# Filippo-Galli/Split_and_merge_Gibbs_sampling

Measured on AMD Instinct MI355X. Metric: full Gibbs sweeps/sec (N-point reassign) at N=1M D=128; achieved HBM GB/s, higher is better.
Workload: dtype f64

## Files before the change

include/hdpm.h:

```cpp
#ifndef HDPM_H
#define HDPM_H

#include <stdint.h>

#ifdef __cplusplus
extern "C" {
#endif

#define HDPM_OK          0
#define HDPM_E_VALIDATE  1
#define HDPM_E_GSL       2
#define HDPM_E_PROB      3
#define HDPM_E_WALKER    4
#define HDPM_E_ARG       5
#define HDPM_E_DEVICE    6
#define HDPM_E_NODEVICE  7

typedef struct hdpm_ctx hdpm_ctx;

typedef struct {
    int32_t verbose, m, iterations, L, burnin, t, r;
    int32_t neal8, split_merge, n8_step_size, sam_step_size, thinning;
} hdpm_chain_params;

typedef struct {
    int64_t sweeps, rounds, restarts, exact_points, moves, checked_rounds, prepass_points;
    double  t_prepass_ms, t_resolve_ms, t_stats_ms, t_host_phi_ms, t_rng_ms, t_loglik_ms, t_exact_ms;
    int64_t pool_calls, pool_entries, pool_device_calls;
    double  t_pool_ms, t_pool_mt_ms, t_pool_accept_ms, t_pool_parse_ms, t_pool_values_ms;
    int64_t phi_spec_runs, phi_spec_clusters;
    int64_t prepass_timed, prepass_timed_points;
    int64_t rng_windows, rng_windows_fresh;
    int64_t listed_points;
    int64_t sm_moves;
    double  t_sm_ms, t_sm_scan_ms, t_sm_phi_ms, t_sm_terms_ms;
    int64_t phi_device_calls, phi_device_fallbacks, phi_device_last_status;
    int64_t phi_lookahead_hits, phi_lookahead_copies;
    int64_t pipe_enqueued, pipe_runs, pipe_refused, pipe_recovered;
    int64_t phi_tree_calls, phi_tree_retries;
    int64_t pool_walk_fallbacks;
    int64_t phi_dspec_launched, phi_dspec_used;
    int64_t fpg_launches;
    int64_t phi_sm_device_calls;
    int64_t phi_fallback_status_mask;
    int64_t phi_sm_window_retries;
    int64_t fpg_aborts;
    int64_t exact_mass_launches, exact_lanes_launches;
    int64_t dense_launches;
    int64_t sm_wide_scans, sm_wide_fallbacks;
    int64_t phi_fast_calls, phi_fast_handbacks;
    int64_t labels_mirrored, labels_downloaded;
    int64_t phi_state_direct;
    int64_t phi_chain_launched, phi_chain_used, phi_chain_dropped;
    int64_t pipe_auto, pipe_desync;
    int64_t sm_chain_runs, sm_chain_scans, sm_chain_resumes;
} hdpm_stats;

int         hdpm_device_count(void);
int         hdpm_ctx_create(int32_t device, hdpm_ctx** out);
void        hdpm_ctx_destroy(hdpm_ctx* ctx);
const char* hdpm_last_error(const hdpm_ctx* ctx);

int hdpm_set_data(hdpm_ctx* ctx, const uint8_t* codes, int32_t n, int32_t d, const int32_t* attrisize,
                  double gamma, const double* v, const double* w);

int hdpm_rng_set_seed(hdpm_ctx* ctx, uint32_t seed);
int hdpm_rng_set_state(hdpm_ctx* ctx, const int32_t* state625);
int hdpm_rng_get_state(const hdpm_ctx* ctx, int32_t* state625);

int hdpm_set_state(hdpm_ctx* ctx, const int32_t* c_i, int32_t K, const double* centers, const double* sigma);
int hdpm_get_state(hdpm_ctx* ctx, int32_t* c_i, int32_t* K, double* centers, double* sigma, int32_t cap);

int hdpm_set_pool(hdpm_ctx* ctx, const double* centers, const double* sigma, int64_t P);
int hdpm_get_pool(hdpm_ctx* ctx, double* centers, double* sigma, int64_t P);
int hdpm_generate_pool(hdpm_ctx* ctx, int64_t P);

int hdpm_neal8_sweep(hdpm_ctx* ctx, int32_t m);

int hdpm_update_phi(hdpm_ctx* ctx, const int32_t* cluster_indexes, int32_t n_idx);

int hdpm_compute_loglikelihood(hdpm_ctx* ctx, double* out);

int hdpm_loglik_matrix(hdpm_ctx* ctx, double* L, int32_t* H);

int hdpm_restricted_gibbs(hdpm_ctx* ctx, const int32_t* S, int32_t nS, int32_t i1, int32_t i2, int32_t t);

int hdpm_logprobgs_c_i(hdpm_ctx* ctx, const int32_t* g_c_i, const int32_t* S, int32_t nS, int32_t i1,
                       int32_t i2, double* out);

int hdpm_split_and_merge(hdpm_ctx* ctx, int32_t t, int32_t r, int32_t idx_1_sm, int32_t* accepted);

int hdpm_run_markov_chain(hdpm_ctx* ctx, const hdpm_chain_params* p, const int32_t* c_i_init,
                          int32_t* out_total_cls, int32_t* out_c_i, double* out_loglik,
                          int32_t* out_accepted, int32_t* final_ass, double* out_time_s);

int hdpm_init_chain(hdpm_ctx* ctx, const hdpm_chain_params* p, const int32_t* c_i_init);
int hdpm_iteration(hdpm_ctx* ctx, const hdpm_chain_params* p, int32_t iter, int32_t* idx_1_sm,
                   int32_t* accepted, double* loglik);
int hdpm_iterations(hdpm_ctx* ctx, const hdpm_chain_params* p, int32_t iter0, int32_t count, int32_t* idx_1_sm,
                    int32_t* accepted, double* loglik);

int hdpm_iterations_record(hdpm_ctx* ctx, const hdpm_chain_params* p, int32_t iter0, int32_t count, int32_t* idx_1_sm,
                           int32_t* accepted, double* loglik, int32_t* total_cls, int32_t* c_i, int32_t* nsaved);
int hdpm_record_take(hdpm_ctx* ctx, double* centers, double* sigmas, int64_t* nrows);

int hdpm_rng_fill_device(hdpm_ctx* ctx, int64_t count, uint32_t* out);
int hdpm_get_stats(const hdpm_ctx* ctx, hdpm_stats* out);
int hdpm_reset_stats(hdpm_ctx* ctx);
// ... 33 lines not shown
```

split_and_merge_gibbs_sampling_amd/_lib.py:

```python
from __future__ import annotations

import ctypes as C
import os
import subprocess

import numpy as np

PKG_DIR = os.path.dirname(os.path.abspath(__file__))
LIB_PATH = os.path.join(PKG_DIR, "libhdpm.so")
if os.environ.get("HDPM_LIB_VARIANT"):
    LIB_PATH = os.path.join(PKG_DIR, f"libhdpm_{os.environ['HDPM_LIB_VARIANT']}.so")
CSRC = os.path.join(PKG_DIR, "csrc")

EXPORTS = (
    "hdpm_device_count", "hdpm_ctx_create", "hdpm_ctx_destroy", "hdpm_last_error", "hdpm_set_data",
    "hdpm_rng_set_seed", "hdpm_rng_set_state", "hdpm_rng_get_state", "hdpm_set_state", "hdpm_get_state",
    "hdpm_set_pool", "hdpm_get_pool", "hdpm_generate_pool", "hdpm_neal8_sweep", "hdpm_update_phi",
    "hdpm_compute_loglikelihood", "hdpm_loglik_matrix", "hdpm_restricted_gibbs", "hdpm_logprobgs_c_i",
    "hdpm_split_and_merge", "hdpm_run_markov_chain", "hdpm_get_stats", "hdpm_reset_stats",
    "hdpm_set_debug", "hdpm_synchronize", "hdpm_drop_prepared", "hdpm_init_chain", "hdpm_iteration", "hdpm_iterations", "hdpm_iterations_record", "hdpm_record_take", "hdpm_rng_fill_device",
    "hdpm_get_pool_heads", "hdpm_set_option", "hdpm_get_option", "hdpm_debug_draw", "hdpm_debug_math",
    "hdpm_psm_build", "hdpm_psm_rows", "hdpm_psm_vi_lb",
    "hdpm_trace_build", "hdpm_trace_terms", "hdpm_trace_losses", "hdpm_trace_tables",
)

OPT_HIG_LOGSPACE = 1
OPT_PHI_DEVICE = 2
OPT_PIPE_WAIT_US = 3
OPT_FPG_WAIT_US = 4
OPT_FPG_FAIL_AT = 5
OPT_EXACT_KERNEL = 6
OPT_LAT_NEGLIGIBLE = 7
OPT_SM_WIDE_WAIT_US = 8
OPT_SM_CHAIN = 9
OPT_CAPTURE_DELAY_US = 10

STATUS = {0: "OK", 1: "E_VALIDATE", 2: "E_GSL", 3: "E_PROB", 4: "E_WALKER", 5: "E_ARG",
          6: "E_DEVICE", 7: "E_NODEVICE"}


class HdpmError(RuntimeError):
    def __init__(self, status: int, msg: str):
        super().__init__(f"hdpm {STATUS.get(status, status)}: {msg}")
        self.status = status


class ChainParams(C.Structure):
    _fields_ = [(n, C.c_int32) for n in (
        "verbose", "m", "iterations", "L", "burnin", "t", "r", "neal8", "split_merge",
        "n8_step_size", "sam_step_size", "thinning")]


class Stats(C.Structure):
    _fields_ = [(n, C.c_int64) for n in (
        "sweeps", "rounds", "restarts", "exact_points", "moves", "checked_rounds", "prepass_points")] + \
        [(n, C.c_double) for n in (
            "t_prepass_ms", "t_resolve_ms", "t_stats_ms", "t_host_phi_ms", "t_rng_ms", "t_loglik_ms",
            "t_exact_ms")] + \
        [(n, C.c_int64) for n in ("pool_calls", "pool_entries", "pool_device_calls")] + \
        [(n, C.c_double) for n in (
            "t_pool_ms", "t_pool_mt_ms", "t_pool_accept_ms", "t_pool_parse_ms", "t_pool_values_ms")] + \
        [(n, C.c_int64) for n in ("phi_spec_runs", "phi_spec_clusters", "prepass_timed", "prepass_timed_points",
                                  "rng_windows", "rng_windows_fresh", "listed_points", "sm_moves")] + \
        [(n, C.c_double) for n in ("t_sm_ms", "t_sm_scan_ms", "t_sm_phi_ms", "t_sm_terms_ms")] + \
        [(n, C.c_int64) for n in ("phi_device_calls", "phi_device_fallbacks", "phi_device_last_status",
                                  "phi_lookahead_hits", "phi_lookahead_copies", "pipe_enqueued", "pipe_runs",
                                  "pipe_refused", "pipe_recovered", "phi_tree_calls", "phi_tree_retries",
                                  "pool_walk_fallbacks", "phi_dspec_launched", "phi_dspec_used",
                                  "fpg_launches", "phi_sm_device_calls", "phi_fallback_status_mask",
                                  "phi_sm_window_retries", "fpg_aborts", "exact_mass_launches",
                                  "exact_lanes_launches", "dense_launches", "sm_wide_scans",
                                  "sm_wide_fallbacks", "phi_fast_calls", "phi_fast_handbacks",
                                  "labels_mirrored", "labels_downloaded", "phi_state_direct",
                                  "phi_chain_launched", "phi_chain_used", "phi_chain_dropped",
                                  "pipe_auto", "pipe_desync", "sm_chain_runs", "sm_chain_scans",
                                  "sm_chain_resumes")]

    def as_dict(self):
        return {k: getattr(self, k) for k, _ in self._fields_}


def build(force: bool = False) -> str:
    srcs = [os.path.join(CSRC, f) for f in os.listdir(CSRC)]
    stale = force or not os.path.exists(LIB_PATH) or \
        max(os.path.getmtime(s) for s in srcs) > os.path.getmtime(LIB_PATH)
    if stale:
        subprocess.run(["make", "-s", "-C", CSRC], check=True)
    return LIB_PATH


_lib = None


def lib():
    global _lib
    if _lib is not None:
        return _lib
    if not os.path.exists(LIB_PATH):
        raise ImportError(f"libhdpm.so not built ({LIB_PATH}); run __graft_entry__.build()")
    L = C.CDLL(LIB_PATH)
    vp, i32, i64, f64 = C.c_void_p, C.c_int32, C.c_int64, C.c_double
    P = C.POINTER
    sig = {
        "hdpm_device_count": ([], C.c_int),
        "hdpm_ctx_create": ([i32, P(vp)], C.c_int),
        "hdpm_ctx_destroy": ([vp], None),
        "hdpm_last_error": ([vp], C.c_char_p),
        "hdpm_set_data": ([vp, vp, i32, i32, vp, f64, vp, vp], C.c_int),
        "hdpm_rng_set_seed": ([vp, C.c_uint32], C.c_int),
        "hdpm_rng_set_state": ([vp, vp], C.c_int),
        "hdpm_rng_get_state": ([vp, vp], C.c_int),
        "hdpm_set_state": ([vp, vp, i32, vp, vp], C.c_int),
        "hdpm_get_state": ([vp, vp, P(i32), vp, vp, i32], C.c_int),
        "hdpm_set_pool": ([vp, vp, vp, i64], C.c_int),
        "hdpm_get_pool": ([vp, vp, vp, i64], C.c_int),
        "hdpm_generate_pool": ([vp, i64], C.c_int),
        "hdpm_neal8_sweep": ([vp, i32], C.c_int),
        "hdpm_update_phi": ([vp, vp, i32], C.c_int),
        "hdpm_compute_loglikelihood": ([vp, P(f64)], C.c_int),
        "hdpm_loglik_matrix": ([vp, vp, vp], C.c_int),
        "hdpm_restricted_gibbs": ([vp, vp, i32, i32, i32, i32], C.c_int),
        "hdpm_logprobgs_c_i": ([vp, vp, vp, i32, i32, i32, P(f64)], C.c_int),
        "hdpm_split_and_merge": ([vp, i32, i32, i32, P(i32)], C.c_int),
        "hdpm_run_markov_chain": ([vp, P(ChainParams), vp, vp, vp, vp, vp, vp, vp], C.c_int),
        "hdpm_get_stats": ([vp, P(Stats)], C.c_int),
        "hdpm_init_chain": ([vp, P(ChainParams), vp], C.c_int),
        "hdpm_iteration": ([vp, P(ChainParams), i32, P(i32), P(i32), P(f64)], C.c_int),
        "hdpm_iterations": ([vp, P(ChainParams), i32, i32, P(i32), vp, vp], C.c_int),
        "hdpm_iterations_record": ([vp, P(ChainParams), i32, i32, P(i32), vp, vp, vp, vp, P(i32)], C.c_int),
# ... 30 lines not shown
```

split_and_merge_gibbs_sampling_amd/csrc/engine.cpp:

```cpp
#include <hip/hip_runtime.h>

#include <algorithm>
#include <cctype>
#include <atomic>
#include <chrono>
#include <condition_variable>
#include <cstdlib>
#include <functional>
#include <mutex>
#include <pthread.h>
#include <sched.h>
#include <dirent.h>
#include <dlfcn.h>
#include <execinfo.h>
#include <csignal>
#include <unistd.h>
#include <cmath>
#include <cstdio>
#include <cstring>
#include <memory>
#include <string>
#include <thread>
#include <unordered_map>
#include <vector>
// ... 727 lines not shown
    DevBuf<int32_t> gj, gn, cidx;
    PinBuf<int64_t> h_starts;
    int64_t walk_fallbacks = 0;
    DevBuf<PoolClass> cls;
    DevBuf<int> runs;
    DevBuf<int32_t> att;
    DevBuf<uint64_t> gtab;
    DevBuf<int> err;
    PinBuf<int> h_err;
  } pg;

  PinBuf<uint32_t> h_raw;
  DevBuf<uint32_t> d_raw;
  DevBuf<double> d_L;
  int Ecap = 0;
  DevBuf<double> d_margin;
  DevBuf<int> d_rowpos;
  DevBuf<int> d_list, d_cnt, d_dense, d_dense_total, d_spec, d_boff;
  DevBuf<double> d_spec_rad;
  DevBuf<int4> d_rq;
  DevBuf<uint64_t> d_csum;
  DevBuf<unsigned> d_hist_part;
  DevBuf<long long> d_rprof;
  DevBuf<int> d_fpg;
  DevBuf<int> d_wide_ctr;
  DevBuf<int> d_warm;
  DevBuf<unsigned int> d_lmask;
  bool kernels_warm = false;
  int fpg_grid_cache[65] = {0};
  int fpg_grid_m = -1;
  int& fpg_grid(int lcap, int m) {
    if (m != fpg_grid_m) {
      std::fill(fpg_grid_cache, fpg_grid_cache + 65, 0);
      fpg_grid_m = m;
    }
    return fpg_grid_cache[lcap];
  }
  PinBuf<int> h_ctl;
  int par = 0;
  hipEvent_t ev_res[2] = {nullptr, nullptr};
  size_t ctl_stride() const { return kCtlInts + 3 * (size_t)scap; }
  ResolveCtl* ctl_at(int q) { return reinterpret_cast<ResolveCtl*>(h_ctl.p + (size_t)q * ctl_stride()); }
  PinBuf<PipeSlot> h_pipe;
  DevBuf<PipeGate> d_pipe;
  struct PreSweep {
    bool active = false;
    bool round_ok = false;
    int par = 0, buf = -1, m = 0;
    bool track = false;
    bool dev = false;
    uint64_t gen[2] = {0, 0};
    std::chrono::steady_clock::time_point t_enq;
    bool au = false;
  } pre;
  bool pipe_auto = true;
  int pre_dev_decision() {
    if (!pre.active || !pre.au) return 0;
    const int* w = &h_pipe.p[pre.par].dev;
    const auto t0 = std::chrono::steady_clock::now();
    for (int polls = 0;; ++polls) {
      const int v = __atomic_load_n(w, __ATOMIC_ACQUIRE);
      if (v != 0) return v;
      HostPool::spin_pause();
      if ((polls & 1023) == 1023 && std::chrono::steady_clock::now() - t0 > std::chrono::seconds(5)) {
        return 2;
      }
    }
  }
  long long pipe_limit_ticks = 200000000LL;
  bool pipe_host_check = true;
  long long fpg_limit_ticks = 200000000LL;
  int fpg_fail_at = 0;
  bool fpg_skip = false;
  int last_xpath = 0;
  int exact_pref = 0;
  double lat_negl = kLatNegligible;
  long long sm_wide_ticks = 5000000;
  int sm_chain_mode = [] {
    const char* e = std::getenv("HDPM_SM_CHAIN");
    return (e && e[0] == '1') ? 1 : 0;
  }();
  bool deep_ok = false;
  static constexpr size_t kCtlInts = 16;
  static_assert(sizeof(ResolveCtl) <= kCtlInts * sizeof(int), "control block");
  PinBuf<uint8_t> h_stage_buf[3];
  hipEvent_t ev_stage_buf[3] = {nullptr, nullptr, nullptr};
  int stage_fill = 0, stage_last = 1;
  int stage_hold = -1;
  struct { bool active = false, dev = false; int buf = 0, nent = 0; } commit_later;
  DevBuf<uint8_t> d_stage;

  DevBuf<unsigned> d_freq, d_freq2, d_freq_m;
  bool freq_dev_valid = false;
  bool recount_only() const { return (debug & 16) != 0; }
  uint64_t freq_d2h_version = 0;
  DevBuf<int> d_mlog, d_mcount;
  PinBuf<unsigned> h_freq;
  DevBuf<unsigned char> d_mask;
  PinBuf<unsigned char> h_mask;
  StreamAhead phi_stream;
  int64_t phi_prefetch = 4096;
  DevBuf<double> d_partial;
  PinBuf<double> h_partial;

  hdpm_stats stats{};
  int64_t launch_count = 0;
  bool round_timed = false, round_fine = false;
  int64_t round_points = 0;
  bool pre_timed[2] = {false, false};
  hipEvent_t ev_pp[2][2] = {{nullptr, nullptr}, {nullptr, nullptr}};
  int debug = 0;
  std::vector<std::pair<const char*, std::chrono::steady_clock::time_point>> trace;
  void mark(const char* what) {
    if (debug & 34) trace.emplace_back(what, std::chrono::steady_clock::now());
  }
  std::vector<std::pair<std::string, double>> trace_sum;
  std::vector<std::vector<float>> trace_smp;
  void trace_add(const std::string& name, double us) {
    size_t q = 0;
    while (q < trace_sum.size() && trace_sum[q].first != name) ++q;
    if (q == trace_sum.size()) {
      trace_sum.emplace_back(name, 0.0);
      trace_smp.emplace_back();
    }
    trace_sum[q].second += us;
    trace_smp[q].push_back((float)us);
  }
  int64_t trace_iters = 0, trace_alloc0 = -1, trace_slow = 0;
  char spec_line[192] = {0};
  std::unordered_map<uint64_t, bool> beta_cache;

  SmWork sm;
  std::vector<double> sp;
  std::vector<int> sperm;

  ~Ctx() {
    PoolScope scope(hpool);
    try {
      cancel_ahead();
    } catch (...) {
    }
// ... 419 lines not shown
      for (int b = 0; b < wb; ++b)
        if ((code >> b) & 1u) out[b * Ws + (j >> 6)] |= 1ull << (j & 63);
      A += (long double)tab[2 * j];
      sc += (long double)std::max(std::fabs(tab[2 * j]), std::fabs(tab[2 * j + 1]));
      const double dj = tab[2 * j] - tab[2 * j + 1];
      dmax = std::max(dmax, dj);
      dmin = std::min(dmin, dj);
    }
    const double delta = dmax > 0 ? dmax / ((1 << kQ) - 1) : 0.0;
    for (int j = 0; j < d; ++j) {
      const double dj = tab[2 * j] - tab[2 * j + 1];
      int q = delta > 0 ? (int)std::floor(dj / delta) : 0;
      q = std::min(std::max(q, 0), (1 << kQ) - 1);
      while (q > 0 && delta * q > dj) --q;
      while (q < (1 << kQ) - 1 && delta * (q + 1) <= dj) ++q;
      for (int b = 0; b < kQ; ++b)
        if ((q >> b) & 1) out[(wb + b) * Ws + (j >> 6)] |= 1ull << (j & 63);
    }
    double* s = reinterpret_cast<double*>(out + (wb + kQ) * Ws);
    s[0] = (double)A;
    s[1] = delta;
    s[2] = dmin > 0 ? dmin : 0.0;
    s[3] = (double)sc;
  }

  void ensure_slots(int need) {
    if (need <= scap) return;
    int nc = std::max(need, std::max(2 * scap, 64));
    d_counts.ensure(nc, true, stream);
    d_sol.ensure(nc, true, stream);
    d_los.ensure(nc, true, stream);
    d_src.ensure(nc, true, stream);
    d_slot_codes.ensure((size_t)nc * dp, true, stream);
    d_slot_tab.ensure((size_t)nc * 2 * d, true, stream);
    d_slot_bnd.ensure((size_t)nc * bw, true, stream);
    d_freq.ensure((size_t)nc * d * mmax, true, stream);
    d_freq2.ensure((size_t)nc * d * mmax);
    scap = nc;
  }

  UploadLayout stage_begin(int nent) {
    const UploadLayout L = upload_layout(nent, dp, d, bw);
    auto pick = [&] {
      int f = 0;
      while (f < 3 && (f == stage_last || f == stage_hold || (commit_later.active && f == commit_later.buf))) ++f;
      return f;
    };
    int f = pick();
    if (f >= 3) {
      flush_commit();
      f = pick();
    }
    stage_fill = f;
    hipEvent_t& ev = ev_stage_buf[stage_fill];
    if (!ev) HIPCHK(hipEventCreateWithFlags(&ev, hipEventDisableTiming));
    HIPCHK(hipEventSynchronize(ev));
    PinBuf<uint8_t>& hb = h_stage_buf[stage_fill];
    if (hb.n < L.bytes) hb.ensure(L.bytes + L.bytes / 2 + 4096, hipHostMallocCoherent);
    d_stage.ensure(L.bytes);
    return L;
  }
  uint8_t* stage_ptr() { return h_stage_buf[stage_fill].p; }
  void stage_entry(const UploadLayout& L, int r, int k) {
    uint8_t* st = stage_ptr();
    double* tt = (double*)(st + L.off_tab) + (size_t)r * 2 * d;
    tables_for(&h_center[(size_t)k * d], &h_sigma[(size_t)k * d], st + L.off_codes + (size_t)r * dp, tt);
    bounds_for(&h_center[(size_t)k * d], tt, (uint64_t*)(st + L.off_bnd) + (size_t)r * bw);
    ((int*)(st + L.off_counts))[r] = h_counts[k];
    ((int*)(st + L.off_slot))[r] = k;
  }
  void stage_commit(const UploadLayout& L, int nent, bool full) {
    if (stage_hold == stage_fill) stage_hold = -1;
    HIPCHK(hipMemcpyAsync(d_stage.p, stage_ptr(), L.bytes, hipMemcpyHostToDevice, stream));
    HIPCHK(hipEventRecord(ev_stage_buf[stage_fill], stream));
    stage_last = stage_fill;
    stage_full = full;
    HIPCHK(launch_scatter_clusters(d_stage.p, nent, dp, d, bw, full ? 1 : 0, d_slot_codes.p, d_slot_tab.p,
                                   d_slot_bnd.p, d_counts.p, d_sol.p, d_los.p, d_src.p, stream));
  }

  bool defer_commit = false;
  void flush_commit() {
    if (!commit_later.active) return;
    commit_later.active = false;
    if (commit_later.dev) {
      commit_later.dev = false;
      scatter_dev_stage(commit_later.nent);
      return;
    }
    stage_fill = commit_later.buf;
    stage_commit(upload_layout(commit_later.nent, dp, d, bw), commit_later.nent, true);
  }

  void stage_upload(const std::vector<int>* which) {
    const int nent = which ? (int)which->size() : K;
    if (nent == 0) return;
    const UploadLayout L = stage_begin(nent);
    pool_for(nent, [&](int r) { stage_entry(L, r, which ? (*which)[r] : r); });
    stage_commit(L, nent, which == nullptr);
  }

  void upload_clusters() {
    ensure_slots(K + 2);
    stage_upload(nullptr);
    tables_dirty = false;
  }
// ... 819 lines not shown
    if (!host_spec()) {
      dspec_launch();
      mark("ahead.dspec");
    }
    if (resolve_smem_bytes(std::min(scap, K + 2), m, K + m <= 64 ? 1 : 0) <= 160 * 1024) {
      par ^= 1;
      ahead.par = par;
      ahead.track = freq_dev_valid;
      sweep_buffers(ahead.track, m);
      mark("ahead.buf");
      if (launch) {
        if (launch_round(0, K, m, ahead.raw, ahead.track) == kOk) ahead.launched = true;
      } else if (!(debug & 131072)) {
        HIPCHK(hipEventRecord(ev[7], stream));
        if (launch_round(0, K, m, ahead.raw, ahead.track, kRoundPrefix) == kOk) ahead.prefix = true;
      }
    }
    if (sweep_first && host_spec()) {
      spec_launch();
      mark("ahead.spec");
    }
  }
  void cancel_ahead() {
    pre_release();
    if (!ahead.active) return;
    ahead.active = false;
    if (ahead.launched) {
      (void)hipStreamSynchronize(stream);
      have_state = false;
      err = "a prepared sweep was abandoned";
    }
    if (spec.ran) {
      if (!spec.joined && pj_open) (void)pj_finish();
      spec.ran = false;
    }
    dspec.ran = false;
    dnext.ran = false;
    phi_stream.n = 0;
    pend.active = false;
    rng = ahead.saved;
  }

  int last_sweep_rounds = 0, last_sweep_moves = -1;

  void pre_enqueue(int m, bool track) {
    const int q = 1 - par;
    if (h_pipe.n < 2) h_pipe.ensure(2, hipHostMallocCoherent);
    d_pipe.ensure(2);
    sweep_buffers(track, m);
    __atomic_store_n(&h_pipe.p[q].flag, 0, __ATOMIC_RELEASE);
    __atomic_store_n(&h_pipe.p[q].dev, 0, __ATOMIC_RELEASE);
    h_pipe.p[q].raw = nullptr;
    h_pipe.p[q].raw_dev = nullptr;
    const bool dev = !host_spec();
    const uint64_t lo = dev ? dspec.pos : spec.pos;
    const uint64_t hi = lo + (uint64_t)(dev ? dspec.pl.need : 2 * phi_prefetch) + (uint64_t)n * (m + 1);
    int whole = -1;
    for (int k = 0; k < 2; ++k) {
      const RngWindow& w = win[k];
      if (w.valid && w.epoch == rng.epoch && w.start_pos <= lo && hi <= w.start_pos + (uint64_t)w.count &&
          (whole < 0 || w.start_pos < win[whole].start_pos))
        whole = k;
    }
    for (int k = 0; k < 2; ++k) {
      pre.gen[k] = ~0ull;
      const RngWindow& w = win[k];
      if (whole >= 0 ? k == whole
                     : (w.valid && w.epoch == rng.epoch && w.start_pos < hi && lo < w.start_pos + (uint64_t)w.count)) {
        HIPCHK(hipStreamWaitEvent(stream, w.done, 0));
        pre.gen[k] = w.gen;
      }
    }
    static const bool auto_env_off = [] {
      const char* e = std::getenv("HDPM_PIPE_AUTO");
      return e && e[0] == '0';
    }();
    PipeAuto au{};
    const bool labels_from_device = record_now && !host_c_valid;
    if (dev && pipe_auto && !auto_env_off && dspec.ran && dspec.fast && dspec.chain && whole >= 0 &&
        !labels_from_device) {
      const RngWindow& w = win[whole];
      au = PipeAuto{dspec.chain, w.raw.p, (int64_t)w.start_pos, w.count, (int64_t)n * (m + 1), 1};
    }
    if (dev) HIPCHK(hipStreamWaitEvent(stream, dspec.ev, 0));
    HIPCHK(launch_pipe_wait(&h_pipe.p[q], ctl_at(par), ctl_at(q), n, &d_pipe.p[q], pipe_limit_ticks, stream, au));
    pre.au = au.on != 0;
    pre.t_enq = std::chrono::steady_clock::now();
    pre.active = true;
    pre.par = q;
    pre.dev = dev;
    pre.buf = dev ? -1 : spec.stage_buf;
    pre.m = m;
    pre.track = track;
    pre.round_ok = false;
    d_csum.ensure((size_t)K * (bw + 2));
    d_wide_ctr.ensure(4);
    int* zero = nullptr;
    if (mcount_clear && K > 0) {
      zero = d_mcount.p;
      mcount_clear = false;
    }
    if (dev) {
      HIPCHK(launch_scatter_clusters(dspec.stage, K, dp, d, bw, 1, d_slot_codes.p, d_slot_tab.p, d_slot_bnd.p,
                                     d_counts.p, d_sol.p, d_los.p, d_src.p, stream, &d_pipe.p[q].gate, d_csum.p,
                                     d_logn.p, zero, d_wide_ctr.p));
      phd_release(stream);
    } else {
      HIPCHK(launch_scatter_clusters(h_stage_buf[pre.buf].p, K, dp, d, bw, 1, d_slot_codes.p, d_slot_tab.p,
                                     d_slot_bnd.p, d_counts.p, d_sol.p, d_los.p, d_src.p, stream, &d_pipe.p[q].gate,
                                     d_csum.p, d_logn.p, zero, d_wide_ctr.p));
    }
    summary_by_scatter = true;
    pre.round_ok = launch_round(0, K, m, nullptr, track, kRoundAll, &d_pipe.p[q], q) == kOk;
    summary_by_scatter = false;
    if (!dev) HIPCHK(hipEventRecord(ev_stage_buf[pre.buf], stream));
    stats.pipe_enqueued++;
  }
  void pre_release() {
    if (!pre.active) return;
    if (pre_dev_decision() == 1) {
      (void)hipStreamSynchronize(stream);
      have_state = false;
      err = "a sweep went ahead on the device after the host released it";
      stats.pipe_desync++;
    }
    pre.active = false;
    __atomic_store_n(&h_pipe.p[pre.par].flag, 2, __ATOMIC_RELEASE);
  }
  bool pipe_go(int m) {
    const bool went = pre_dev_decision() == 1;
    const bool agree = pre.active && pre.round_ok && pre.m == m && commit_later.active && last_sweep_rounds == 1 &&
                       last_sweep_moves == 0 && !tables_dirty;
    if (went && !(agree && pre.dev && commit_later.dev && freq_dev_valid && freq_version == labels_version)) {
      (void)hipStreamSynchronize(stream);
      have_state = false;
      err = "a sweep went ahead on the device where the host would not have";
      stats.pipe_desync++;
      pre.active = false;
      return false;
    }
    if (!went) {
      if (!agree) return false;
      if (pre.dev ? (!commit_later.dev || !dspec_on()) : (commit_later.dev || commit_later.buf != pre.buf || !host_spec()))
        return false;
      if (!(freq_dev_valid && freq_version == labels_version)) return false;
      if (pipe_host_check &&
          std::chrono::duration<double, std::micro>(std::chrono::steady_clock::now() - pre.t_enq).count() >
              (double)pipe_limit_ticks * 0.01 * 0.25) {
        stats.pipe_refused++;
        return false;
      }
    }
    rng_sync();
    const Rng saved = rng;
    const uint32_t* raw = device_draws((int64_t)n * (m + 1));
    PipeSlot& sl = h_pipe.p[pre.par];
    if (went) {
      raw = __atomic_load_n(&sl.raw_dev, __ATOMIC_ACQUIRE);
      stats.pipe_auto++;
    } else {
      bool waited = false;
      for (int k = 0; k < 2; ++k)
        if (win[k].gen == pre.gen[k] && raw >= win[k].raw.p && raw < win[k].raw.p + win[k].count) waited = true;
      if (!waited) {
        pend.active = false;
        phidev.valid = false;
        rng = saved;
        return false;
      }
      __atomic_store_n(&sl.raw, raw, __ATOMIC_RELAXED);
      __atomic_store_n(&sl.flag, 1, __ATOMIC_RELEASE);
    }
    pre.active = false;
    mark("go");
    ahead.saved = saved;
    ahead.raw = raw;
    ahead.m = m;
    ahead.lv = labels_version;
    ahead.launched = true;
    ahead.prefix = false;
    ahead.track = pre.track;
    ahead.par = pre.par;
    ahead.piped = true;
    ahead.active = true;
    stats.prepass_points += n;
    stats.pipe_runs++;
    commit_later.active = false;
    if (pre.dev) {
      commit_later.dev = false;
      stage_full = false;
      if (!dspec_promote(m)) dspec_launch();
      dnext_launch(m);
    } else {
      stage_last = pre.buf;
      stage_full = true;
      if (stage_hold == pre.buf) stage_hold = -1;
      spec_launch();
    }
    mark("ahead.spec");
    return true;
  }

  int neal8_sweep(int m) {
    const bool use_ahead = ahead.active && ahead.m == m && ahead.lv == labels_version && !tables_dirty;
    if (!use_ahead) cancel_ahead();
    if (!have_state) { err = "no state"; return kArg; }
    if (P <= 0) { err = "no latent pool"; return kArg; }
    if (m <= 0) { err = "m must be positive"; return kArg; }
    {
      if (!host_c_valid || host_c_device) {  }
      else {
        std::vector<char> seen(K + 1, 0);
        int u = 0;
        for (int i = 0; i < n; ++i) {
          const int c = h_c[i];
          if (c >= K) { cancel_ahead(); err = "State validation failed: inconsistent cluster count"; return kValidate; }
          if (!seen[c]) { seen[c] = 1; u++; }
        }
        if (u != K) { cancel_ahead(); err = "State validation failed: inconsistent cluster count"; return kValidate; }
      }
    }
    if (tables_dirty) upload_clusters();
    const bool spec_go = freq_dev_valid && freq_version == labels_version && !(debug & 128) && !recount_only() &&
                         host_spec();
    const bool freq_before_ok = freq_version == labels_version && !recount_only();
    const bool dspec_go = freq_dev_valid && freq_version == labels_version && !recount_only() && dspec_on();
    if (!use_ahead) {
      spec.ran = false;
      dspec.ran = false;
    }
    spec.lv = 0;
    labels_version++;
    const int K0 = K;
    int sweep_moves = 0;
    const bool hc_before = host_c_valid;
    std::vector<uint8_t> old_center = h_center;
    std::vector<double> old_sigma = h_sigma;

    auto tr0 = std::chrono::steady_clock::now();
    const size_t nraw = (size_t)n * (m + 1);
    const uint32_t* d_sweep_raw = use_ahead ? ahead.raw : device_draws((int64_t)nraw);
    const bool ahead_launched = use_ahead && ahead.launched;
    const bool ahead_prefix = use_ahead && ahead.prefix && !ahead.launched;
    const bool ahead_piped = ahead_launched && ahead.piped;
    if (ahead_launched || ahead_prefix) par = ahead.par;
    else par ^= 1;
    ahead.active = false;
    mark("draws");
    struct SpecGuard {
      Ctx* c;
      ~SpecGuard() {
        if (c->spec.ran && !c->spec.joined && c->pj_open) {
          (void)c->pj_finish();
          c->spec.ran = false;
        }
      }
    } spec_guard{this};
    if (spec_go && !use_ahead) spec_launch();
    else if (dspec_go && !use_ahead) dspec_launch();
    stats.t_rng_ms += std::chrono::duration<double, std::milli>(std::chrono::steady_clock::now() - tr0).count();

    int nslots = K;
    int p = 0;
    bool end_queued = false;
    const int64_t rounds0 = stats.rounds;
    const bool launched_ahead = ahead_launched;
    const bool track = (launched_ahead || ahead_prefix) ? ahead.track : (freq_dev_valid && !recount_only());
    if (!launched_ahead && !ahead_prefix) sweep_buffers(track, m);
    while (p < n) {
      if (!(launched_ahead && stats.rounds == rounds0)) {
        const int part = (ahead_prefix && stats.rounds == rounds0) ? kRoundResolve : kRoundAll;
        const int lst = launch_round(p, nslots, m, d_sweep_raw, track, part);
        if (lst) return lst;
        end_queued = last_sweep_moves > 0;
        if (end_queued) launch_sweep_end(scap - 2, track);
      } else {
        end_queued = false;
      }
      mark("launched");
      if (stats.rounds == rounds0) {
        if (deep_ok && (host_spec() ? (spec.ran && spec.K == K) : (dspec.ran && dspec.K == K)) && track &&
            last_sweep_moves == 0 && !(debug & 4194304)) {
          pre_enqueue(m, track);
          mark("pre");
        }
        if (spec.ran) spec_join();
        else if (host_spec()) prefill_phi_stream();
      }
      mark("prefill");
      HIPCHK(hipEventSynchronize(ev_res[par]));
      mark("resolved");
      const bool piped_round = ahead_piped && stats.rounds == rounds0;
      if (piped_round ? pre_timed[par] : round_timed) {
        float t1 = 0;
        if (piped_round) round_points = n;
        HIPCHK(hipEventElapsedTime(&t1, piped_round ? ev_pp[par][0] : ev[0], piped_round ? ev_pp[par][1] : ev[1]));
        stats.t_prepass_ms += t1;
        stats.prepass_timed++;
        stats.prepass_timed_points += round_points;
      }
      if (round_fine && !piped_round) {
        float t2 = 0, t3 = 0;
        HIPCHK(hipEventElapsedTime(&t3, ev[1], ev[5]));
        HIPCHK(hipEventElapsedTime(&t2, ev[5], ev[2]));
        stats.t_exact_ms += t3;
        stats.t_resolve_ms += t2;
      }
      stats.rounds++;
      const ResolveCtl c = *ctl_at(par);
      if (c.status == kPipeOff && piped_round) {
        if (pre.dev || stage_last < 0 || !stage_full) {
          upload_clusters();
        } else {
          stage_fill = stage_last;
          stage_commit(upload_layout(K, dp, d, bw), K, true);
        }
        if (track) mcount_clear = true;
        stats.pipe_recovered++;
        continue;
      }
      if (pre.active && (c.status || c.next < n || c.moves)) pre_release();
      last_sweep_rounds = (int)(stats.rounds - rounds0);
      if ((debug & 2) && last_fp && last_fpg) {
        long long tp[16];
        HIPCHK(hipMemcpy(tp, d_rprof.p, sizeof(tp), hipMemcpyDeviceToHost));
        std::fprintf(stderr,
                     "[resolve_fpg] G %d: %lld listed in %lld windows, %lld rounds; init %.2f us, rounds %.2f us, drift / "
                     "re-test / commit %.2f us, in grid barriers %.2f us, total %.2f us\n",
                     last_fpg, tp[9], tp[8], tp[5], (tp[1] - tp[0]) / 100.0, tp[3] / 100.0, tp[4] / 100.0, tp[2] / 100.0,
                     (tp[7] - tp[0]) / 100.0);
      } else if ((debug & 2) && last_fp) {
        long long tp[16];
        HIPCHK(hipMemcpy(tp, d_rprof.p, sizeof(tp), hipMemcpyDeviceToHost));
        std::fprintf(stderr,
                     "[resolve_fp] init %.2f us, %lld listed in %lld chunks: rounds %lld (%.2f us), drift / re-test / "
                     "commit %.2f us, %lld stops (%.2f us), total %.2f us; in rounds: counts %.2f us, ballots %.2f us, "
                     "evaluations (slowest wave) %.2f us, %lld evaluations, %lld own draws (row loads + draws: %.2f us, summed over waves)\n",
                     (tp[1] - tp[0]) / 100.0, tp[9], tp[8], tp[5], tp[3] / 100.0, tp[4] / 100.0, tp[6], tp[2] / 100.0,
                     (tp[7] - tp[0]) / 100.0, tp[10] / 100.0, tp[11] / 100.0, tp[12] / 100.0, tp[14], tp[15], tp[13] / 100.0);
      } else if (debug & 2) {
        long long tp[16];
        HIPCHK(hipMemcpy(tp, d_rprof.p, sizeof(tp), hipMemcpyDeviceToHost));
        std::fprintf(stderr,
                     "[resolve] init %.2f us, batches %.2f us, decided points %lld in %.2f us (exact decisions "
                     "%.2f us, state updates %.2f us, re-tests %.2f us over %lld points; block mode: %lld blocks), "
                     "total %.2f us\n",
                     (tp[1] - tp[0]) / 100.0, tp[3] / 100.0, tp[6], tp[4] / 100.0, tp[12] / 100.0, tp[14] / 100.0,
                     tp[13] / 100.0, tp[15], tp[5], (tp[7] - tp[0]) / 100.0);
      }
      stats.exact_points += c.exact;
      stats.listed_points += c.listed;
      last_exact = c.exact;
      last_listed = c.listed;
      if (p == 0 || last_density < 0)
        last_density = (double)(c.uncertain >= 0 ? c.uncertain : c.listed) / (double)std::max(1, n - p);
      stats.moves += c.moves;
      sweep_moves += c.moves;
      stats.checked_rounds += c.checked;
      last_unsettled = c.checked || (c.restart && c.next < n);
      if (c.aborted && !c.status) {
        stats.fpg_aborts++;
        fpg_skip = true;
// ... 1752 lines not shown
  }
  h_center.assign((size_t)K * d, 0);
  h_sigma.assign((size_t)K * d, 0.0);
  for (int k = 0; k < K; ++k) sample_center_uniform(&h_center[(size_t)k * d]);
  for (int k = 0; k < K; ++k) {
    int st = sample_sigma(v.data(), w.data(), &h_sigma[(size_t)k * d]);
    if (st) { err = "rhig failed"; return st; }
  }
  recount();
  upload_labels();
  upload_clusters();
  have_state = true;
  int st = update_phi(nullptr, 0);
  if (st) return st;
  return generate_pool((int64_t)n * p->m * p->thinning);
}

int Ctx::iteration(const hdpm_chain_params* p, int iter, int* idx_1_sm, int* accepted, double* ll, bool launch_next,
                   int32_t* labels_out) {
  int st;
  *accepted = 0;
  trace.clear();
  mark("start");
  const bool n8 = p->neal8 && iter % p->n8_step_size == 0;
  const bool sm_now = p->split_merge && iter % p->sam_step_size == 0;
  const bool next_n8 = p->neal8 && (iter + 1) % p->n8_step_size == 0;
  const bool early = n8 && !sm_now && next_n8 && iter % 1000 != 0 && !(debug & 2097152);
  if (!n8) cancel_ahead();
  if (n8) {
    deep_ok = early && launch_next && !(debug & 4194304);
    record_now = labels_out != nullptr;
    st = neal8_sweep(p->m);
    deep_ok = false;
    record_now = false;
    if (st) {
      pre_release();
      return st;
    }
    if (labels_out) capture_labels();
    defer_commit = early;
    st = update_phi(nullptr, 0);
    defer_commit = false;
    if (st) {
      pre_release();
      flush_commit();
      return st;
    }
  }
  bool prepared = false;
  if (pre.active) {
    if (early && launch_next && pipe_go(p->m)) prepared = true;
    else pre_release();
  }
  if (!prepared && early && commit_later.active && freq_version == labels_version && !(debug & 4) && !tables_dirty) {
    prepare_next_sweep(p->m, launch_next);
    prepared = true;
  }
  flush_commit();
  if (sm_now) {
    const auto t0 = std::chrono::steady_clock::now();
    st = split_and_merge(p->t, p->r, *idx_1_sm, accepted);
    stats.t_sm_ms += std::chrono::duration<double, std::milli>(std::chrono::steady_clock::now() - t0).count();
    stats.sm_moves++;
    if (st) return st;
    *idx_1_sm = (*idx_1_sm + 1) % n;
  }
  if (iter % 1000 == 0) {
    st = generate_pool((int64_t)n * p->m * p->thinning);
    if (st) return st;
  }
  st = compute_loglikelihood(ll);
  mark("loglik");
  if (!st && labels_out) {
    if (sm_now || !n8) capture_labels();
    std::memcpy(labels_out, h_c.data(), (size_t)n * 4);
  }
  if (!st && next_n8 && !prepared) {
    prepare_next_sweep(p->m, launch_next);
    prepared = true;
  }
  if (prepared && ahead.active && host_spec()) phi_lookahead();
  mark("ahead");
  if ((debug & 32) && trace.size() > 1) {
    if (trace_alloc0 < 0) trace_alloc0 = g_dev_allocs.load();
    for (size_t k = 1; k < trace.size(); ++k) {
      const double us = std::chrono::duration<double, std::micro>(trace[k].second - trace[k - 1].second).count();
      trace_add(trace[k].first, us);
    }
    const double tot = std::chrono::duration<double, std::micro>(trace.back().second - trace.front().second).count();
    trace_add("total", tot);
    if (tot > 180.0 && trace_slow++ < 12) {
      std::string line = "[slow iteration " + std::to_string(trace_iters) + "]";
      for (size_t k = 1; k < trace.size(); ++k) {
        char buf[64];
        std::snprintf(buf, sizeof(buf), " %s %.0f", trace[k].first,
                      std::chrono::duration<double, std::micro>(trace[k].second - trace[k - 1].second).count());
        line += buf;
      }
      std::fprintf(stderr, "%s%s\n", line.c_str(), spec_line);
    }
    trace_iters++;
  }
  if ((debug & 2) && trace.size() > 1) {
    std::string line = "[iter]";
    for (size_t k = 1; k < trace.size(); ++k) {
      char buf[96];
// ... 752 lines not shown
```

split_and_merge_gibbs_sampling_amd/csrc/kernels.hip:

```cpp
#include <hip/hip_runtime.h>

#include <algorithm>
#include <cfloat>
#include <cmath>
#include <cstdlib>
#include <cstdio>

#include "glibc_math.hpp"
#include "kernels.hpp"

namespace hdpm {

int device_cus() {
  static int cache[64] = {0};
  int dev = 0;
  if (hipGetDevice(&dev) != hipSuccess || dev < 0 || dev >= 64) dev = 0;
  int c = __atomic_load_n(&cache[dev], __ATOMIC_RELAXED);
  if (c <= 0) {
    if (hipDeviceGetAttribute(&c, hipDeviceAttributeMultiprocessorCount, dev) != hipSuccess || c <= 0) c = 256;
    __atomic_store_n(&cache[dev], c, __ATOMIC_RELAXED);
  }
  return c;
}

// ... 3781 lines not shown
  } else if (a.fp) {
    const size_t lds = resolve_fp_lds_bytes(a.lcap, a.m);
    if (a.K + a.m <= 24) HDPM_LAUNCH(k_resolve_fp<24>, dim3(1), dim3(kFpThreads), lds, s, a);
    else if (a.K + a.m <= 32) HDPM_LAUNCH(k_resolve_fp<32>, dim3(1), dim3(kFpThreads), lds, s, a);
    else HDPM_LAUNCH(k_resolve_fp<64>, dim3(1), dim3(kFpThreads), lds, s, a);
  } else if (a.blocks)
    HDPM_LAUNCH(k_resolve_blk, dim3(1), dim3(kWave), resolve_lds_bytes(a.lcap, a.m, 1), s, a);
  else
    HDPM_LAUNCH(k_resolve, dim3(1), dim3(kWave), resolve_lds_bytes(a.lcap, a.m, 0, a.S + a.m), s, a);
  return hipGetLastError();
}

hipError_t launch_relabel(int* c, const int* los, int n, const ResolveCtl* ctl, hipStream_t s) {
  HDPM_LAUNCH(k_relabel, dim3((n + kBlock - 1) / kBlock), dim3(kBlock), 0, s, c, los, n, ctl);
  return hipGetLastError();
}

hipError_t launch_apply_moves(const int* mlog, const int* mcount, int grid, const uint8_t* codes_t, int d, int nq,
                              int mmax, unsigned int* freq, const ResolveCtl* ctl, int n, int nslots, hipStream_t s) {
  const int ls = std::min(nslots, (int)(64 * 1024 / ((size_t)d * mmax * 4)));
  if (ls >= 2) {
    HDPM_LAUNCH(k_apply_moves_lds, dim3(512), dim3(256), (size_t)ls * d * mmax * 4, s, mlog, mcount, codes_t, d,
                       nq, mmax, freq, ctl, n, ls);
    return hipGetLastError();
  }
  HDPM_LAUNCH(k_apply_moves, dim3(std::max(1, std::min(grid, 4096))), dim3(kWave), 0, s, mlog, mcount, codes_t,
                     d, nq, mmax, freq, ctl, n);
  return hipGetLastError();
}

hipError_t launch_freq_gather(const unsigned int* freq, const int* sol, int Kmax, int fs, unsigned int* out,
                              const ResolveCtl* ctl, int n, hipStream_t s) {
  const int64_t work = (int64_t)std::max(Kmax, 1) * fs;
  HDPM_LAUNCH(k_freq_gather, dim3((unsigned)std::min<int64_t>(1024, (work + 255) / 256)), dim3(256), 0, s, freq,
                     sol, fs, out, ctl, n);
  return hipGetLastError();
}

hipError_t launch_finish_sweep(int* counts, int* sol, int* los, int* src, int cap, const ResolveCtl* ctl, int n,
                               hipStream_t s) {
  HDPM_LAUNCH(k_finish_sweep, dim3(1), dim3(1024), (size_t)(2 * cap) * 4, s, counts, sol, los, src, ctl, n);
  return hipGetLastError();
}

__global__ void k_pipe_wait(PipeSlot* slot, const ResolveCtl* prev, ResolveCtl* own, int n, PipeGate* g,
                            long long limit, PipeAuto au) {
  if (threadIdx.x != 0) return;
  if (au.on) {
    const volatile ResolveCtl* c = prev;
    const int cok = __hip_atomic_load(&au.chain->ok, __ATOMIC_ACQUIRE, __HIP_MEMORY_SCOPE_AGENT);
    const int64_t end =
        (int64_t)__hip_atomic_load(reinterpret_cast<const uint64_t*>(&au.chain->end), __ATOMIC_RELAXED, __HIP_MEMORY_SCOPE_AGENT);
    const int64_t r = end - au.win_start;
    const bool ok = cok == 1 && c->status == 0 && c->next >= n && c->moves == 0 && r >= 0 && r + au.sweep_len <= au.win_count;
    if (ok) {
      const uint32_t* raw = au.win_raw + r;
      g->raw = raw;
      g->status = 4;
      g->gate = 1;
      __hip_atomic_store(reinterpret_cast<uint64_t*>(&slot->raw_dev), reinterpret_cast<uint64_t>(raw), __ATOMIC_RELAXED,
                         __HIP_MEMORY_SCOPE_SYSTEM);
      __hip_atomic_store(&slot->dev, 1, __ATOMIC_RELEASE, __HIP_MEMORY_SCOPE_SYSTEM);
      return;
    }
    __hip_atomic_store(&slot->dev, 2, __ATOMIC_RELEASE, __HIP_MEMORY_SCOPE_SYSTEM);
  }
  const long long t0 = wall_clock64();
  int f = 0;
  for (;;) {
    f = __hip_atomic_load(&slot->flag, __ATOMIC_RELAXED, __HIP_MEMORY_SCOPE_SYSTEM);
    if (f != 0) {
      __builtin_amdgcn_fence(__ATOMIC_ACQUIRE, "");
      break;
    }
    if (wall_clock64() - t0 > limit) {
      f = 3;
      break;
    }
    __builtin_amdgcn_s_sleep(8);
  }
  const volatile ResolveCtl* c = prev;
  const bool ok = f == 1 && c->status == 0 && c->next >= n && c->moves == 0;
  const uint64_t rw =
      __hip_atomic_load(reinterpret_cast<const uint64_t*>(&slot->raw), __ATOMIC_ACQUIRE, __HIP_MEMORY_SCOPE_SYSTEM);
  g->raw = ok ? reinterpret_cast<const uint32_t*>(rw) : nullptr;
  g->status = f;
  g->gate = ok ? 1 : 0;
  if (!ok) {
    volatile ResolveCtl* o = own;
    o->status = kPipeOff;
    o->next = 0;
    o->aborted = 0;
    o->uncertain = -1;
  }
}
hipError_t launch_pipe_wait(PipeSlot* slot, const ResolveCtl* prev, ResolveCtl* own, int n, PipeGate* g,
                            long long limit, hipStream_t s, const PipeAuto& au) {
  HDPM_LAUNCH(k_pipe_wait, dim3(1), dim3(64), 0, s, slot, prev, own, n, g, limit, au);
  return hipGetLastError();
}

hipError_t launch_scatter_clusters(const uint8_t* stage, int nent, int dp, int d, int bw, int full, uint8_t* codes,
                                   double* tab, uint64_t* bnd, int* counts, int* sol, int* los, int* src,
                                   hipStream_t s, const int* gate, uint64_t* csum, const double* logn, int* zero,
                                   int* wide_ctr) {
  if (csum && !full) return hipErrorInvalidValue;
  const int64_t work = (int64_t)nent * std::max(2 * d, std::max(dp, bw + 2));
  const int nb = (int)std::max<int64_t>(1, std::min<int64_t>(1024, (work + 255) / 256));
  const ScatterSummary sum{csum, logn, zero, wide_ctr};
  HDPM_LAUNCH(k_scatter_clusters, dim3(nb), dim3(256), 0, s, stage, nent, dp, d, bw, full, codes, tab, bnd,
                     counts, sol, los, src, gate, sum);
  return hipGetLastError();
}

size_t hist_partial_words(const HistArgs& a, int* nbx_out, int* kc_out, int* tpb_out) {
  const int64_t per_label = (int64_t)a.mmax * a.d * 4;
  const int64_t budget = 96 * 1024 - (int64_t)(kHistBlock / kWave) * a.W * 64 * 8 - per_label;
  const int kc = budget > 0 ? (int)std::min<int64_t>(a.K, budget / per_label) : 0;
  const int64_t ntiles = ((int64_t)a.n + 63) / 64;
  const int tpb = (int)std::max<int64_t>(16, (ntiles + 255) / 256);
  const int nbx = (int)((ntiles + tpb - 1) / tpb);
  *nbx_out = nbx;
  *kc_out = kc;
  *tpb_out = tpb;
  if (kc <= 0 || a.W > 8) return 0;
  const int ny = (a.K + kc - 1) / kc;
  return (size_t)ny * nbx * kc * a.mmax * a.d;
}

hipError_t launch_hist(const HistArgs& a0, hipStream_t s) {
  HistArgs a = a0;
  int nbx, kc, tpb;
  const size_t pw = hist_partial_words(a, &nbx, &kc, &tpb);
  const hipError_t e = hipMemsetAsync(a.freq, 0, (size_t)a.K * a.d * a.mmax * 4, s);
  if (e != hipSuccess) return e;
  if (pw > 0 && a.partial && a.xpk) {
    a.KC = kc;
    a.tiles_per_block = tpb;
    const int ny = (a.K + kc - 1) / kc;
    const size_t hbytes = (((size_t)(kc + 1) * a.mmax * a.d * 4 + 15) / 16) * 16;
    const size_t lds = hbytes + (size_t)(kHistBlock / kWave) * a.W * 64 * 8;
    HDPM_LAUNCH(k_hist_packed, dim3(nbx, ny), dim3(kHistBlock), lds, s, a);
    const int hsize = kc * a.mmax * a.d;
    HDPM_LAUNCH(k_hist_reduce, dim3((hsize + 255) / 256, ny, kHistReduceSplit), dim3(256), 0, s, a, nbx);
  } else {
    const int64_t nt = (int64_t)a.n * a.nq;
    HDPM_LAUNCH(k_hist_global, dim3((nt + kBlock - 1) / kBlock), dim3(kBlock), 0, s, a);
// ... 776 lines not shown
```

Measured before the change: 8060.

## Release the enqueued-ahead host-spec sweep early, before the current round resolves

Adds an early-go path for the host-speculation pipeline. When the host has already prepared the next sweep's phi stream and reserved its RNG window, it sets the wait slot's flag and raw pointer right after enqueueing, so the device's pipe_wait kernel can proceed without a later host round-trip. The wait kernel now reports its decision in the slot in the non-auto case as well, and staging-buffer reuse is guarded by tracking which pipe slot still reads each buffer. The added consistency checks (draw-pointer match, quiet-sweep confirmation, desync handling) cost extra host logic and risk invalidating state whenever the speculation disagrees with what the host later computes.

```diff
diff --git a/include/hdpm.h b/include/hdpm.h
--- a/include/hdpm.h
+++ b/include/hdpm.h
@@ -54,6 +54,7 @@
     int64_t phi_chain_launched, phi_chain_used, phi_chain_dropped;
     int64_t pipe_auto, pipe_desync;
     int64_t sm_chain_runs, sm_chain_scans, sm_chain_resumes;
+    int64_t pipe_early, pipe_early_ran, pipe_early_off;
 } hdpm_stats;
 
 int         hdpm_device_count(void);
diff --git a/split_and_merge_gibbs_sampling_amd/_lib.py b/split_and_merge_gibbs_sampling_amd/_lib.py
--- a/split_and_merge_gibbs_sampling_amd/_lib.py
+++ b/split_and_merge_gibbs_sampling_amd/_lib.py
@@ -74,7 +74,7 @@
                                   "labels_mirrored", "labels_downloaded", "phi_state_direct",
                                   "phi_chain_launched", "phi_chain_used", "phi_chain_dropped",
                                   "pipe_auto", "pipe_desync", "sm_chain_runs", "sm_chain_scans",
-                                  "sm_chain_resumes")]
+                                  "sm_chain_resumes", "pipe_early", "pipe_early_ran", "pipe_early_off")]
 
     def as_dict(self):
         return {k: getattr(self, k) for k, _ in self._fields_}
diff --git a/split_and_merge_gibbs_sampling_amd/csrc/engine.cpp b/split_and_merge_gibbs_sampling_amd/csrc/engine.cpp
--- a/split_and_merge_gibbs_sampling_amd/csrc/engine.cpp
+++ b/split_and_merge_gibbs_sampling_amd/csrc/engine.cpp
@@ -803,18 +803,29 @@
     uint64_t gen[2] = {0, 0};
     std::chrono::steady_clock::time_point t_enq;
     bool au = false;
+    bool early = false;
+    const uint32_t* early_raw = nullptr;
+    bool early_went = false;
   } pre;
   bool pipe_auto = true;
   int pre_dev_decision() {
-    if (!pre.active || !pre.au) return 0;
-    const int* w = &h_pipe.p[pre.par].dev;
+    if (!pre.active || !(pre.au || pre.early)) return 0;
+    return slot_dev_decision(pre.par);
+  }
+  int slot_dev_decision(int q) {
+    const int* w = &h_pipe.p[q].dev;
     const auto t0 = std::chrono::steady_clock::now();
     for (int polls = 0;; ++polls) {
       const int v = __atomic_load_n(w, __ATOMIC_ACQUIRE);
       if (v != 0) return v;
       HostPool::spin_pause();
       if ((polls & 1023) == 1023 && std::chrono::steady_clock::now() - t0 > std::chrono::seconds(5)) {
-        return 2;
+        (void)hipStreamSynchronize(stream);
+        have_state = false;
+        err = "the wait kernel of a sweep enqueued ahead did not report its decision";
+        stats.pipe_desync++;
+        const int v2 = __atomic_load_n(w, __ATOMIC_ACQUIRE);
+        return v2 != 0 ? v2 : 2;
       }
     }
   }
@@ -838,6 +849,7 @@
   hipEvent_t ev_stage_buf[3] = {nullptr, nullptr, nullptr};
   int stage_fill = 0, stage_last = 1;
   int stage_hold = -1;
+  int stage_pipe_busy[3] = {0, 0, 0};
   struct { bool active = false, dev = false; int buf = 0, nent = 0; } commit_later;
   DevBuf<uint8_t> d_stage;
 
@@ -1363,6 +1375,12 @@
       f = pick();
     }
     stage_fill = f;
+    if (stage_pipe_busy[f]) {
+      const int q = stage_pipe_busy[f] - 1;
+      if (ev_res[q]) HIPCHK(hipEventSynchronize(ev_res[q]));
+      else HIPCHK(hipStreamSynchronize(stream));
+      stage_pipe_busy[f] = 0;
+    }
     hipEvent_t& ev = ev_stage_buf[stage_fill];
     if (!ev) HIPCHK(hipEventCreateWithFlags(&ev, hipEventDisableTiming));
     HIPCHK(hipEventSynchronize(ev));
@@ -2288,6 +2306,9 @@
     __atomic_store_n(&h_pipe.p[q].dev, 0, __ATOMIC_RELEASE);
     h_pipe.p[q].raw = nullptr;
     h_pipe.p[q].raw_dev = nullptr;
+    pre.early = false;
+    pre.early_raw = nullptr;
+    pre.early_went = false;
     const bool dev = !host_spec();
     const uint64_t lo = dev ? dspec.pos : spec.pos;
     const uint64_t hi = lo + (uint64_t)(dev ? dspec.pl.need : 2 * phi_prefetch) + (uint64_t)n * (m + 1);
@@ -2349,8 +2370,39 @@
     summary_by_scatter = true;
     pre.round_ok = launch_round(0, K, m, nullptr, track, kRoundAll, &d_pipe.p[q], q) == kOk;
     summary_by_scatter = false;
-    if (!dev) HIPCHK(hipEventRecord(ev_stage_buf[pre.buf], stream));
+    if (!dev) stage_pipe_busy[pre.buf] = q + 1;
     stats.pipe_enqueued++;
+  }
+  void pipe_early_go(int m, bool track, bool freq_before_ok) {
+    static const bool env_off = [] {
+      const char* e = std::getenv("HDPM_PIPE_EARLY");
+      return e && e[0] == '0';
+    }();
+    if (env_off || !pre.active || !pre.round_ok || pre.dev || pre.au || pre.m != m) return;
+    if (!pipe_host_check || (record_now && !host_c_valid)) return;
+    const StreamAhead& sa = phi_stream;
+    if (!(deep_ok && host_spec() && !(debug & 128))) return;
+    if (!(spec.ran && spec.joined && K > 0 && spec.K == K && spec.nvalid == K)) return;
+    if (!(spec.pos == rng.pos && spec.epoch == rng.epoch && sa.n > 0 && sa.start.pos == spec.pos)) return;
+    if (!(spec.stage_buf >= 0 && spec.stage_buf == stage_hold && spec.stage_buf == pre.buf)) return;
+    if (!(track && freq_dev_valid && freq_before_ok)) return;
+    if (std::chrono::duration<double, std::micro>(std::chrono::steady_clock::now() - pre.t_enq).count() >
+        (double)pipe_limit_ticks * 0.01 * 0.25)
+      return;
+    const uint64_t pos = spec.pos + (uint64_t)spec.off[K];
+    const int64_t len = (int64_t)n * (m + 1);
+    int wk = -1;
+    for (int k = 0; k < 2; ++k)
+      if (covers(win[k], pos, len) && (wk < 0 || win[k].start_pos < win[wk].start_pos)) wk = k;
+    if (wk < 0 || win[wk].gen != pre.gen[wk]) return;
+    const uint32_t* raw = win[wk].raw.p + (pos - win[wk].start_pos);
+    PipeSlot& sl = h_pipe.p[pre.par];
+    pre.early = true;
+    pre.early_raw = raw;
+    __atomic_store_n(&sl.raw, raw, __ATOMIC_RELAXED);
+    __atomic_store_n(&sl.flag, 1, __ATOMIC_RELEASE);
+    stats.pipe_early++;
+    mark("early_go");
   }
   void pre_release() {
     if (!pre.active) return;
@@ -2362,12 +2414,16 @@
     }
     pre.active = false;
     __atomic_store_n(&h_pipe.p[pre.par].flag, 2, __ATOMIC_RELEASE);
+    if (pre.buf >= 0) stage_pipe_busy[pre.buf] = 0;
   }
   bool pipe_go(int m) {
-    const bool went = pre_dev_decision() == 1;
+    const bool early = pre.active && pre.early;
+    const bool went = early ? pre.early_went : pre_dev_decision() == 1;
     const bool agree = pre.active && pre.round_ok && pre.m == m && commit_later.active && last_sweep_rounds == 1 &&
                        last_sweep_moves == 0 && !tables_dirty;
-    if (went && !(agree && pre.dev && commit_later.dev && freq_dev_valid && freq_version == labels_version)) {
+    const bool same_tables = pre.dev ? (pre.au && commit_later.dev)
+                                     : (pre.early && !commit_later.dev && commit_later.buf == pre.buf && host_spec());
+    if (went && !(agree && same_tables && freq_dev_valid && freq_version == labels_version)) {
       (void)hipStreamSynchronize(stream);
       have_state = false;
       err = "a sweep went ahead on the device where the host would not have";
@@ -2391,7 +2447,16 @@
     const Rng saved = rng;
     const uint32_t* raw = device_draws((int64_t)n * (m + 1));
     PipeSlot& sl = h_pipe.p[pre.par];
-    if (went) {
+    if (went && early) {
+      if (raw != pre.early_raw) {
+        (void)hipStreamSynchronize(stream);
+        have_state = false;
+        err = "a sweep went ahead on the device with other draws than the host reserved";
+        stats.pipe_desync++;
+        pre.active = false;
+        return false;
+      }
+    } else if (went) {
       raw = __atomic_load_n(&sl.raw_dev, __ATOMIC_ACQUIRE);
       stats.pipe_auto++;
     } else {
@@ -2432,9 +2497,17 @@
       stage_full = true;
       if (stage_hold == pre.buf) stage_hold = -1;
       spec_launch();
+      if (early) pipe_early_confirm(pre.par);
     }
     mark("ahead.spec");
     return true;
+  }
+  void pipe_early_confirm(int q) {
+    if (slot_dev_decision(q) == 1 && have_state) return;
+    (void)hipStreamSynchronize(stream);
+    have_state = false;
+    err = "the host followed an early go that the device did not take";
+    stats.pipe_desync++;
   }
 
   int neal8_sweep(int m) {
@@ -2504,6 +2577,7 @@
     const bool track = (launched_ahead || ahead_prefix) ? ahead.track : (freq_dev_valid && !recount_only());
     if (!launched_ahead && !ahead_prefix) sweep_buffers(track, m);
     while (p < n) {
+      bool enqueued = false;
       if (!(launched_ahead && stats.rounds == rounds0)) {
         const int part = (ahead_prefix && stats.rounds == rounds0) ? kRoundResolve : kRoundAll;
         const int lst = launch_round(p, nslots, m, d_sweep_raw, track, part);
@@ -2519,13 +2593,17 @@
             last_sweep_moves == 0 && !(debug & 4194304)) {
           pre_enqueue(m, track);
           mark("pre");
+          enqueued = true;
         }
         if (spec.ran) spec_join();
         else if (host_spec()) prefill_phi_stream();
+        if (enqueued) pipe_early_go(m, track, freq_before_ok);
       }
       mark("prefill");
       HIPCHK(hipEventSynchronize(ev_res[par]));
       mark("resolved");
+      for (int& b : stage_pipe_busy)
+        if (b == par + 1) b = 0;
       const bool piped_round = ahead_piped && stats.rounds == rounds0;
       if (piped_round ? pre_timed[par] : round_timed) {
         float t1 = 0;
@@ -2544,6 +2622,25 @@
       }
       stats.rounds++;
       const ResolveCtl c = *ctl_at(par);
+      if (pre.active && pre.early && enqueued) {
+        if (!c.status && c.next >= n && !c.moves) {
+          pre.early_went = true;
+          stats.pipe_early_ran++;
+        } else {
+          const int dv = pre_dev_decision();
+          pre.active = false;
+          if (pre.buf >= 0) stage_pipe_busy[pre.buf] = 0;
+          if (!have_state) return kArg;
+          if (dv == 1) {
+            (void)hipStreamSynchronize(stream);
+            have_state = false;
+            err = "a sweep went ahead on the device behind a sweep that was not quiet";
+            stats.pipe_desync++;
+            return kArg;
+          }
+          stats.pipe_early_off++;
+        }
+      }
       if (c.status == kPipeOff && piped_round) {
         if (pre.dev || stage_last < 0 || !stage_full) {
           upload_clusters();
@@ -4402,6 +4499,7 @@
     if (early && launch_next && pipe_go(p->m)) prepared = true;
     else pre_release();
   }
+  if (!have_state) return kArg;
   if (!prepared && early && commit_later.active && freq_version == labels_version && !(debug & 4) && !tables_dirty) {
     prepare_next_sweep(p->m, launch_next);
     prepared = true;
diff --git a/split_and_merge_gibbs_sampling_amd/csrc/kernels.hip b/split_and_merge_gibbs_sampling_amd/csrc/kernels.hip
--- a/split_and_merge_gibbs_sampling_amd/csrc/kernels.hip
+++ b/split_and_merge_gibbs_sampling_amd/csrc/kernels.hip
@@ -3857,7 +3857,9 @@
     const int64_t end =
         (int64_t)__hip_atomic_load(reinterpret_cast<const uint64_t*>(&au.chain->end), __ATOMIC_RELAXED, __HIP_MEMORY_SCOPE_AGENT);
     const int64_t r = end - au.win_start;
-    const bool ok = cok == 1 && c->status == 0 && c->next >= n && c->moves == 0 && r >= 0 && r + au.sweep_len <= au.win_count;
+    const int f0 = __hip_atomic_load(&slot->flag, __ATOMIC_RELAXED, __HIP_MEMORY_SCOPE_SYSTEM);
+    const bool ok = f0 != 2 && cok == 1 && c->status == 0 && c->next >= n && c->moves == 0 && r >= 0 &&
+                    r + au.sweep_len <= au.win_count;
     if (ok) {
       const uint32_t* raw = au.win_raw + r;
       g->raw = raw;
@@ -3898,6 +3900,7 @@
     o->aborted = 0;
     o->uncertain = -1;
   }
+  if (!au.on) __hip_atomic_store(&slot->dev, ok ? 1 : 2, __ATOMIC_RELEASE, __HIP_MEMORY_SCOPE_SYSTEM);
 }
 hipError_t launch_pipe_wait(PipeSlot* slot, const ResolveCtl* prev, ResolveCtl* own, int n, PipeGate* g,
                             long long limit, hipStream_t s, const PipeAuto& au) {
```

Result: faster. 8502, median of 6 (+5.5%).
